# cg-tuwien/ppsurf

Hardware: AMD Instinct MI355X
Metric: occupancy query-points/sec @ res=257, 50NN (higher is better)
Workload: dtype f16x3

## Files before the change

### ppsurf_amd/csrc/pps_decode.hip

```cpp
#include <cstdlib>
#include "pps_common.h"
#include "../../include/ppsurf_amd.h"

using namespace pps;

#ifndef NT
#define NT 256
#endif
#define NW (NT / 64)
#ifndef WG_PER_CU
#define WG_PER_CU (512 / NT)
#endif
#ifndef PPS_PRIO
#define PPS_PRIO 1
#endif
#ifndef PPS_PRIO_PN
#define PPS_PRIO_PN 1
#endif
#define CH4 2048

template <int CHUNK_F4_NEXT, int NTH = NT, class F>
__device__ __forceinline__ void stream_step(const f32x4* __restrict__ gnext, f32x4*& cur, f32x4*& nxt, F&& compute) {
    chunk_copy_async<CHUNK_F4_NEXT / NTH, NTH>(gnext, nxt);
    compute((const f32x4*)cur);
// ... 799 lines not shown
                           [&](const f32x4* w) { dense_blocks<8, 4, 1>(h, u[t], w, bias_g + 32, lane); });
        }
#pragma unroll 1
        for (int c = 0; c < 32; ++c) {
            f32x4 o[PB_T][8];
            const f32x4* gn = (c + 1 < 32) ? wg + (6 + c) * CH4 : wg;
            stream_step<CH4>(gn, cur, nxt, [&](const f32x4* w) {
#pragma unroll
                for (int t = 0; t < PB_T; ++t) dense_blocks<4, 8, 0>(u[t], o[t], w, bias4 + 32 * c, lane);
            });
#pragma unroll
            for (int t = 0; t < PB_T; ++t) {
                if (qvs[t]) {
                    f32x4* dst = (f32x4*)(trans2 + qcs[t] * 4096) + g;
#pragma unroll
                    for (int j = 0; j < 8; ++j) dst[4 * (8 * c + j)] = o[t][j];
                }
            }
        }
    }
}

__global__ __launch_bounds__(NT, 2) void pointnet_stn_fc_h_kernel(const float* __restrict__ gin, int64_t Q, const f32x4* __restrict__ w16,
                                                                  const float* __restrict__ bias, half8* __restrict__ trans2h, int* __restrict__ range) {
    float amax = 0.f;
    f32x4* buf0 = (f32x4*)pps_smem;
    f32x4* buf1 = buf0 + CH4;
    float* bias_l = (float*)(buf1 + CH4);
    const f32x4* bias4 = (const f32x4*)bias_l;
    const f32x4* wg = w16;
    const int lane = lane_id(), wave = threadIdx.x >> 6, n = lane & 15, g = lane >> 4;

    lds_fill(bias_l, bias + 192, 4096);
    const f32x4* bias_g = (const f32x4*)bias;
    stream_prologue<CH4>(wg, buf0);
    stream_wait();
    __syncthreads();
    f32x4 *cur = buf0, *nxt = buf1;
    const int ntiles = (int)((Q + NW * 16 - 1) / (NW * 16));
    int first, count, stride;
    xcd_tile_range(ntiles, first, count, stride);
    for (int it = 0; it < count; ++it) {
        const int64_t qi = (int64_t)(first + it * stride) * (NW * 16) + wave * 16 + n;
        const bool qv = qi < Q;
        const int64_t qc = qv ? qi : Q - 1;
        HiLo ah[8], h[4], u[2];
        {
            f32x4 a[16];
            const f32x4* src = (const f32x4*)(gin + qc * 256) + g;
#pragma unroll
            for (int bb = 0; bb < 16; ++bb) a[bb] = src[4 * bb];
#pragma unroll
            for (int kb = 0; kb < 8; ++kb) ah[kb] = split_f16_r(amax, a[2 * kb], a[2 * kb + 1]);
        }
#pragma unroll
        for (int c = 0; c < 4; ++c)
            stream_step<CH4>(wg + (c + 1) * CH4, cur, nxt, [&](const f32x4* w) {
                dense_blocks_f16x3<8, 2, 1>(ah, (const half8*)w, bias_g + 8 * c, lane, [&](int, const f32x4& o0, const f32x4& o1) { h[c] = split_f16_r(amax, o0, o1); }); });
        stream_step<CH4>(wg + 5 * CH4, cur, nxt, [&](const f32x4* w) {
            dense_blocks_f16x3<4, 4, 1>(h, (const half8*)w, bias_g + 32, lane, [&](int i, const f32x4& o0, const f32x4& o1) { u[i] = split_f16_r(amax, o0, o1); }); });
        half8* dst = trans2h + qc * 1024 + g;
#pragma unroll 1
        for (int c = 0; c < 32; ++c) {
            const f32x4* gn = (c + 1 < 32) ? wg + (6 + c) * CH4 : wg;
            stream_step<CH4>(gn, cur, nxt, [&](const f32x4* w) {
                dense_blocks_f16x3<2, 8, 0, false>(u, (const half8*)w, bias4 + 32 * c, lane, [&](int i, const f32x4& o0, const f32x4& o1) {
                    const int a = 2 * c + (i >> 1), kb = i & 1;
                    const HiLo v = split_f16_r(amax, o0, o1);
                    if (qv) {
                        half8* d = dst + (((a >> 4) * 2 + kb) * 2) * 64 + 4 * (a & 15);
                        d[0] = v.hi;
                        d[64] = v.lo;
                    }
                }); });
        }
    }
    range_commit(amax, range);
}

#define PC_W_XYZ 256
#define PC_NBIAS (576 + 256 + 4)
#define PC_WFLOATS (4096 + 8192)
#define PC_LDS_BYTES ((PC_WFLOATS + PC_W_XYZ + PC_NBIAS) * 4)

template <bool H>
__global__ __launch_bounds__(PNT, 2) void pointnet_feat_rows_kernel(const float* __restrict__ patches, const float* __restrict__ trans2,
                                                                    int64_t Q, int P, const float* __restrict__ wpack,
                                                                    const f32x4* __restrict__ wdense, const float* __restrict__ bias,
                                                                    float* __restrict__ xbar, int* __restrict__ flag) {
    if (!H && gate_closed(flag)) return;
    float amax = 0.f;
    f32x4* w_l = (f32x4*)pps_smem;
    float* xyz_l = (float*)(w_l + PC_WFLOATS / 4);
    float* bias_l = xyz_l + PC_W_XYZ;
    const f32x4* bias4 = (const f32x4*)bias_l;
    const f32x4* u4 = bias4 + 144;
    const int lane = lane_id(), wave = threadIdx.x >> 6, n = lane & 15, g = lane >> 4;
    for (int i = threadIdx.x; i < PC_WFLOATS / 4; i += PNT) w_l[i] = wdense[i];
    lds_fill(xyz_l, wpack, PC_W_XYZ);
    lds_fill(bias_l, bias, PC_NBIAS);
    __syncthreads();
    const float s0 = bias_l[576 + 256];
    const f32x4* w_c0b = w_l;
    const f32x4* w_c2 = w_l + 1024;
    const int ntile_rows = (P + 15) / 16;

    const int ntiles = (int)((Q + PNW - 1) / PNW);
    int first, count, stride;
    xcd_tile_range(ntiles, first, count, stride);
    for (int it = 0; it < count; ++it) {
        const int64_t q = (int64_t)(first + it * stride) * PNW + wave;
        if (q >= Q) continue;
        half8 th[4][2], tl[4][2];
        f32x4 tf[4][4];
        if (H) {
            const half8* tq = (const half8*)trans2 + q * 1024 + 4 * n + g;
#pragma unroll
            for (int ob = 0; ob < 4; ++ob)
#pragma unroll
                for (int kb = 0; kb < 2; ++kb) { th[ob][kb] = tq[((ob * 2 + kb) * 2) * 64]; tl[ob][kb] = tq[((ob * 2 + kb) * 2 + 1) * 64]; }
        } else {
            const f32x4* tq = (const f32x4*)(trans2 + q * 4096);
#pragma unroll
            for (int ob = 0; ob < 4; ++ob)
#pragma unroll
                for (int kb = 0; kb < 4; ++kb) tf[ob][kb] = tq[(16 * ob + n) * 16 + 4 * kb + g];
        }
        f32x4 acc[8];
        float mrun = -INFINITY, ssum = 0.f;
#pragma unroll
        for (int bb = 0; bb < 8; ++bb) acc[bb] = f32x4{0.f, 0.f, 0.f, 0.f};
        for (int rb = 0; rb < ntile_rows; ++rb) {
            const int rowi = rb * 16 + n;
            const bool valid = rowi < P;
            const int rowc = valid ? rowi : P - 1;
            const float coord = (g < 3) ? patches[(q * P + rowc) * 3 + g] : 0.f;
            f32x4 x0[4], y[8];
#pragma unroll
            for (int bb = 0; bb < 4; ++bb) x0[bb] = bias4[4 * bb + g];
            xyz_blocks<4>(coord, x0, xyz_l, lane);
            relu_blocks<4>(x0);
            __builtin_amdgcn_s_setprio(PPS_PRIO_PN);
            float s = 0.f;
            if (H) {
                HiLo a[2], b[2];
                a[0] = split_f16_r(amax, x0[0], x0[1]);
                a[1] = split_f16_r(amax, x0[2], x0[3]);
                dense_blocks_f16x3<2, 4, 1>(a, (const half8*)w_c0b, bias4 + 16, lane, [&](int i, const f32x4& o0, const f32x4& o1) { b[i] = split_f16_r(amax, o0, o1); });
#pragma unroll
                for (int ob = 0; ob < 4; ++ob) {
                    f32x4 o = bias4[32 + 4 * ob + g], c = {0.f, 0.f, 0.f, 0.f};
#pragma unroll
                    for (int kb = 0; kb < 2; ++kb) {
                        o = __builtin_amdgcn_mfma_f32_16x16x32_f16(th[ob][kb], b[kb].hi, o, 0, 0, 0);
                        c = __builtin_amdgcn_mfma_f32_16x16x32_f16(th[ob][kb], b[kb].lo, c, 0, 0, 0);
                        c = __builtin_amdgcn_mfma_f32_16x16x32_f16(tl[ob][kb], b[kb].hi, c, 0, 0, 0);
                    }
                    o += c;
#pragma unroll
                    for (int r = 0; r < 4; ++r) x0[ob][r] = fmaxf(o[r], 0.f);
                }
                a[0] = split_f16_r(amax, x0[0], x0[1]);
                a[1] = split_f16_r(amax, x0[2], x0[3]);
                dense_blocks_f16x3<2, 8, 1>(a, (const half8*)w_c2, bias4 + 48, lane, [&](int i, const f32x4& o0, const f32x4& o1) {
                    const f32x4 w0 = u4[4 * (2 * i) + g], w1 = u4[4 * (2 * i + 1) + g];
#pragma unroll
                    for (int r = 0; r < 4; ++r) s += w0[r] * o0[r] + w1[r] * o1[r];
                    y[2 * i] = o0;
                    y[2 * i + 1] = o1;
                });
            } else {
                f32x4 x1[4];
                dense_blocks<4, 4, 1>(x0, x1, w_c0b, bias4 + 16, lane);
#pragma unroll
                for (int ob = 0; ob < 4; ++ob) {
                    f32x4 o = bias4[32 + 4 * ob + g];
#pragma unroll
                    for (int kb = 0; kb < 4; ++kb) {
                        o = __builtin_amdgcn_mfma_f32_16x16x4f32(tf[ob][kb].x, x1[kb].x, o, 0, 0, 0);
                        o = __builtin_amdgcn_mfma_f32_16x16x4f32(tf[ob][kb].y, x1[kb].y, o, 0, 0, 0);
                        o = __builtin_amdgcn_mfma_f32_16x16x4f32(tf[ob][kb].z, x1[kb].z, o, 0, 0, 0);
                        o = __builtin_amdgcn_mfma_f32_16x16x4f32(tf[ob][kb].w, x1[kb].w, o, 0, 0, 0);
                    }
#pragma unroll
                    for (int r = 0; r < 4; ++r) x0[ob][r] = fmaxf(o[r], 0.f);
                }
                dense_blocks<4, 8, 1>(x0, y, w_c2, bias4 + 48, lane);
#pragma unroll
                for (int bb = 0; bb < 8; ++bb) {
                    const f32x4 w4 = u4[4 * bb + g];
#pragma unroll
                    for (int r = 0; r < 4; ++r) s += w4[r] * y[bb][r];
                }
            }
            __builtin_amdgcn_s_setprio(0);
            s += __shfl_xor(s, 16);
            s += __shfl_xor(s, 32);
            s += s0;
            const float mblk = row16_max(valid ? s : -INFINITY);
            const float mnew = fmaxf(mrun, mblk);
            const float scale = __expf(mrun - mnew);
            const float en = valid ? __expf(s - mnew) : 0.f;
            mrun = mnew;
            ssum = ssum * scale + en;
#pragma unroll
            for (int bb = 0; bb < 8; ++bb)
#pragma unroll
                for (int r = 0; r < 4; ++r) acc[bb][r] = acc[bb][r] * scale + en * y[bb][r];
        }
        const float inv = 1.f / row16_sum(ssum);
        rows16_sum_transposed8(acc, lane);
        if (n < 8) ((f32x4*)(xbar + q * 128))[4 * n + g] = acc[0] * inv;
    }
    if (H) range_commit(amax, flag);
}

#define TL_NBIAS (256 + 256 + 32)
#define TL_LDS_BYTES (2 * CH4 * 16 + TL_NBIAS * 4)

__global__ __launch_bounds__(NT, 2) void decode_tail_kernel(const float* __restrict__ pooled, const float* __restrict__ xbar, int64_t Q,
                                                            const float* __restrict__ wpack, const float* __restrict__ bias,
                                                            float* __restrict__ logits, float* __restrict__ occ, int* __restrict__ gate) {
    if (gate_closed(gate)) return;
    if (gate != nullptr && blockIdx.x == 0 && threadIdx.x == 0) atomicAdd(gate + 1, 1);
    f32x4* buf0 = (f32x4*)pps_smem;
    f32x4* buf1 = buf0 + CH4;
    float* bias_l = (float*)(buf1 + CH4);
    const f32x4* bias4 = (const f32x4*)bias_l;
    const f32x4* wg = (const f32x4*)wpack;
    const int lane = lane_id(), wave = threadIdx.x >> 6, n = lane & 15, g = lane >> 4;

    lds_fill(bias_l, bias, TL_NBIAS);
    stream_prologue<CH4>(wg, buf0);
    stream_wait();
    __syncthreads();
    f32x4 *cur = buf0, *nxt = buf1;

    const int ntiles = (int)((Q + NW * 16 - 1) / (NW * 16));
    int first, count, stride;
    xcd_tile_range(ntiles, first, count, stride);
    for (int it = 0; it < count; ++it) {
        const int64_t qi = (int64_t)(first + it * stride) * (NW * 16) + wave * 16 + n;
        const bool qv = qi < Q;
        const int64_t qc = qv ? qi : Q - 1;
        f32x4 p[16], x[8], h[16];
        {
            const f32x4* sp = (const f32x4*)(pooled + qc * 256) + g;
            const f32x4* sx = (const f32x4*)(xbar + qc * 128) + g;
#pragma unroll
            for (int bb = 0; bb < 16; ++bb) p[bb] = sp[4 * bb];
#pragma unroll
            for (int bb = 0; bb < 8; ++bb) x[bb] = sx[4 * bb];
        }
#pragma unroll
        for (int c = 0; c < 8; ++c)
            stream_step<CH4>(wg + (c + 1) * CH4, cur, nxt,
                           [&](const f32x4* w) { dense_blocks<16, 2, 0>(p, &h[2 * c], w, bias4 + 8 * c, lane); });
#pragma unroll
        for (int c = 0; c < 4; ++c)
            stream_step<CH4>(wg + (c + 9) * CH4, cur, nxt,
                           [&](const f32x4* w) { dense_blocks<8, 4, 1, 1>(x, &h[4 * c], w, bias4, lane); });
#pragma unroll
        for (int c = 0; c < 8; ++c)
            stream_step<CH4>(wg + (c + 13) * CH4, cur, nxt,
                           [&](const f32x4* w) { dense_blocks<16, 2, 1>(h, &p[2 * c], w, bias4 + 64 + 8 * c, lane); });
        f32x4 o[2];
        stream_step<CH4>(wg, cur, nxt, [&](const f32x4* w) { dense_blocks<16, 2, 0>(p, o, w, bias4 + 128, lane); });
        if (qv && g == 0) {
            const float l0 = o[0].x, l1 = o[0].y;
            logits[qi * 2] = l0;
            logits[qi * 2 + 1] = l1;
            if (occ) {
                const float mx = fmaxf(l0, l1);
                const float e0 = __expf(l0 - mx), e1 = __expf(l1 - mx);
                occ[qi] = (e0 - e1) / (e0 + e1);
            }
        }
    }
}

__global__ __launch_bounds__(NT, 2) void decode_tail_h_kernel(const float* __restrict__ pooled, const float* __restrict__ xbar, int64_t Q,
                                                              const f32x4* __restrict__ w16, const float* __restrict__ bias,
                                                              float* __restrict__ logits, float* __restrict__ occ, int* __restrict__ range) {
    float amax = 0.f;
    f32x4* buf0 = (f32x4*)pps_smem;
    f32x4* buf1 = buf0 + CH4;
    float* bias_l = (float*)(buf1 + CH4);
    const f32x4* bias4 = (const f32x4*)bias_l;
    const f32x4* wg = w16;
    const int lane = lane_id(), wave = threadIdx.x >> 6, n = lane & 15, g = lane >> 4;

    lds_fill(bias_l, bias, TL_NBIAS);
    stream_prologue<CH4>(wg, buf0);
    stream_wait();
    __syncthreads();
    f32x4 *cur = buf0, *nxt = buf1;

// ... 20 lines not shown
            stream_step<CH4 / 2>(wg + c * 3072 + 2048, cur, nxt, [&](const f32x4* w) {
                dense_blocks_f16x3<8, 2, 0>(p, (const half8*)w, bias4 + 8 * c, lane, [&](int, const f32x4& o0, const f32x4& o1) { h[0] = o0; h[1] = o1; }); });
            stream_step<CH4>(c + 1 < 8 ? wg + (c + 1) * 3072 : wg + 24576, cur, nxt, [&](const f32x4* w) {
                dense_blocks_f16x3<4, 2, 1, true, true>(x, (const half8*)w, bias4, lane, [&](int, const f32x4& o0, const f32x4& o1) { y[c] = split_f16_r(amax, o0, o1); }, h); });
        }
#pragma unroll
        for (int c = 0; c < 8; ++c)
            stream_step<CH4>(wg + 24576 + (c + 1) * 2048, cur, nxt, [&](const f32x4* w) {
                dense_blocks_f16x3<8, 2, 1>(y, (const half8*)w, bias4 + 64 + 8 * c, lane, [&](int, const f32x4& o0, const f32x4& o1) { p[c] = split_f16_r(amax, o0, o1); }); });
        f32x4 o[2];
        stream_step<CH4>(wg, cur, nxt, [&](const f32x4* w) {
            dense_blocks_f16x3<8, 2, 0>(p, (const half8*)w, bias4 + 128, lane, [&](int, const f32x4& o0, const f32x4& o1) { o[0] = o0; o[1] = o1; }); });
        if (qv && g == 0) {
            const float l0 = o[0].x, l1 = o[0].y;
            logits[qi * 2] = l0;
            logits[qi * 2 + 1] = l1;
            if (occ) {
                const float mx = fmaxf(l0, l1);
                const float e0 = __expf(l0 - mx), e1 = __expf(l1 - mx);
                occ[qi] = (e0 - e1) / (e0 + e1);
            }
        }
    }
    range_commit(amax, range);
}

static int g_cu_count = 0;
static int cu_count() {
    if (g_cu_count == 0) {
        int dev = 0;
        hipDeviceProp_t prop;
        if (hipGetDevice(&dev) != hipSuccess || hipGetDeviceProperties(&prop, dev) != hipSuccess) return -1;
        g_cu_count = prop.multiProcessorCount;
    }
    return g_cu_count;
}

template <class K>
static int set_lds(K kernel, int bytes) {
    return hipFuncSetAttribute((const void*)kernel, hipFuncAttributeMaxDynamicSharedMemorySize, bytes) == hipSuccess ? 0 : 1;
}

static int grid_for(int64_t ntiles) {
    int cus = cu_count();
    if (cus <= 0) cus = 256;
    cus *= WG_PER_CU;
    return (int)(ntiles < cus ? (ntiles > 0 ? ntiles : 1) : cus);
}

struct PnSplit { int64_t q_packed; int grid_packed, grid_rest, rest_mode; };
static PnSplit pn_split(int64_t q, int p) {
    int cus = cu_count();
    if (cus <= 0) cus = 256;
    const PatchPacking pk = patch_packing(p);
    PnSplit sp;
    const int wgs = cus * PN_WG_PER_CU;
    const int64_t per_round = (int64_t)wgs * PNW * pk.qg;
    sp.q_packed = pk.packed ? (q / per_round) * per_round : 0;
    if (pk.packed && getenv("PPS_PN_FORCE_PACK")) sp.q_packed = q;
    sp.grid_packed = wgs;
    sp.rest_mode = pk.packed ? 2 : 0;
    const int64_t rest_tiles = (q - sp.q_packed + PNW - 1) / PNW;
    sp.grid_rest = (int)(rest_tiles < wgs ? rest_tiles : wgs);
    return sp;
}

#define PPS_LAUNCH_CHECK() (hipGetLastError() == hipSuccess ? PPS_OK : PPS_ERR_LAUNCH)

template <bool H>
static int launch_stn_rows(const float* patches, int64_t q, int p, const float* wpack, const void* wdense, const float* bias, float* g,
                           int* flag, void* stream) {
    static int once = set_lds(pointnet_stn_rows_kernel<H>, PA_LDS_BYTES);
    (void)once;
    const PnSplit sp = pn_split(q, p);
    if (sp.q_packed > 0)
        hipLaunchKernelGGL(pointnet_stn_rows_kernel<H>, dim3(sp.grid_packed), dim3(PNT), PA_LDS_BYTES, (hipStream_t)stream, patches,
                           sp.q_packed, p, 1, wpack, (const f32x4*)wdense, bias, g, flag);
    if (q > sp.q_packed)
        hipLaunchKernelGGL(pointnet_stn_rows_kernel<H>, dim3(sp.grid_rest), dim3(PNT), PA_LDS_BYTES, (hipStream_t)stream,
                           patches + sp.q_packed * p * 3, q - sp.q_packed, p, sp.rest_mode, wpack, (const f32x4*)wdense, bias, g + sp.q_packed * 256, flag);
    return PPS_LAUNCH_CHECK();
}

template <bool H>
static int launch_feat_rows(const float* patches, const float* trans2, int64_t q, int p, const float* wpack, const void* wdense,
                            const float* bias, float* xbar, int* flag, void* stream) {
    static int once = set_lds(pointnet_feat_rows_kernel<H>, PC_LDS_BYTES);
    (void)once;
    int cus = cu_count();
    if (cus <= 0) cus = 256;
    const int64_t ntiles = (q + PNW - 1) / PNW, wgs = (int64_t)cus * PN_WG_PER_CU;
    hipLaunchKernelGGL(pointnet_feat_rows_kernel<H>, dim3((unsigned)(ntiles < wgs ? ntiles : wgs)), dim3(PNT), PC_LDS_BYTES, (hipStream_t)stream, patches,
                       trans2, q, p, wpack, (const f32x4*)wdense, bias, xbar, flag);
    return PPS_LAUNCH_CHECK();
}


static int interp_pool_f32_impl(const float* G, const float* pts, const float* query, const int64_t* idx, int64_t q, int k,
                                const float* wpack, const float* bias, float* pooled, const int* gate, void* stream) {
    if (q < 0 || k < 1 || k > 64) return PPS_ERR_ARG;
    if (q == 0) return PPS_OK;
    if (!G || !pts || !query || !idx || !wpack || !bias || !pooled) return PPS_ERR_ARG;
    static int once = set_lds(interp_pool_kernel, IP_LDS_BYTES);
    (void)once;
    hipLaunchKernelGGL(interp_pool_kernel, dim3(grid_for((q + NW / 4 - 1) / (NW / 4))), dim3(NT), IP_LDS_BYTES, (hipStream_t)stream,
                       G, pts, query, idx, q, k, wpack, bias, pooled, gate);
    return PPS_LAUNCH_CHECK();
}

static int stn_fc_f32_impl(const float* g, int64_t q, const float* wpack, const float* bias, float* trans2, const int* gate, void* stream) {
    if (q < 0) return PPS_ERR_ARG;
    if (q == 0) return PPS_OK;
    if (!g || !wpack || !bias || !trans2) return PPS_ERR_ARG;
    static int once = set_lds(pointnet_stn_fc_kernel, PB_LDS_BYTES);
    (void)once;
    hipLaunchKernelGGL(pointnet_stn_fc_kernel, dim3(grid_for((q + NW * 16 * PB_T - 1) / (NW * 16 * PB_T))), dim3(NT), PB_LDS_BYTES, (hipStream_t)stream,
                       g, q, wpack, bias, trans2, gate);
    return PPS_LAUNCH_CHECK();
}

static int decode_tail_f32_impl(const float* pooled, const float* xbar, int64_t q, const float* wpack, const float* bias,
                                float* logits, float* occ, int* gate, void* stream) {
    if (q < 0) return PPS_ERR_ARG;
    if (q == 0) return PPS_OK;
    if (!pooled || !xbar || !wpack || !bias || !logits) return PPS_ERR_ARG;
    static int once = set_lds(decode_tail_kernel, TL_LDS_BYTES);
    (void)once;
    hipLaunchKernelGGL(decode_tail_kernel, dim3(grid_for((q + NW * 16 - 1) / (NW * 16))), dim3(NT), TL_LDS_BYTES, (hipStream_t)stream,
                       pooled, xbar, q, wpack, bias, logits, occ, gate);
    return PPS_LAUNCH_CHECK();
}

extern "C" {

int pps_abi_version(void) { return 2; }

int pps_debug_occupancy(int which) {
    int n = -1;
    if (which == 0) { set_lds(interp_pool_kernel, IP_LDS_BYTES); hipOccupancyMaxActiveBlocksPerMultiprocessor(&n, interp_pool_kernel, NT, IP_LDS_BYTES); }
    if (which == 1) { set_lds(pointnet_stn_rows_kernel<false>, PA_LDS_BYTES); hipOccupancyMaxActiveBlocksPerMultiprocessor(&n, pointnet_stn_rows_kernel<false>, PNT, PA_LDS_BYTES); }
    if (which == 3) { set_lds(pointnet_stn_fc_kernel, PB_LDS_BYTES); hipOccupancyMaxActiveBlocksPerMultiprocessor(&n, pointnet_stn_fc_kernel, NT, PB_LDS_BYTES); }
    if (which == 4) { set_lds(pointnet_stn_fc_h_kernel, PB_LDS_BYTES); hipOccupancyMaxActiveBlocksPerMultiprocessor(&n, pointnet_stn_fc_h_kernel, NT, PB_LDS_BYTES); }
    if (which == 2) { set_lds(pointnet_feat_rows_kernel<false>, PC_LDS_BYTES); hipOccupancyMaxActiveBlocksPerMultiprocessor(&n, pointnet_feat_rows_kernel<false>, PNT, PC_LDS_BYTES); }
    return n;
}
int pps_device_cu_count(void) { return cu_count(); }

int pps_rows_dense256_f32(const float* in, int64_t rs, int64_t cs, int64_t m, const float* wpack, const float* bias,
                          float* out, void* stream) {
    if (m < 0) return PPS_ERR_ARG;
    if (m == 0) return PPS_OK;
    if (!in || !wpack || !bias || !out) return PPS_ERR_ARG;
    if (cs == 1 && (rs % 4) != 0) return PPS_ERR_ARG;
    static int once = set_lds(rows_dense256_kernel, RD_LDS_BYTES);
    (void)once;
    hipLaunchKernelGGL(rows_dense256_kernel, dim3(grid_for((m + NW * 16 - 1) / (NW * 16))), dim3(NT), RD_LDS_BYTES, (hipStream_t)stream,
                       in, rs, cs, m, wpack, bias, out);
    return PPS_LAUNCH_CHECK();
}

int pps_interp_pool_f32(const float* G, const float* pts, const float* query, const int64_t* idx, int64_t q, int k,
                        const float* wpack, const float* bias, float* pooled, void* stream) {
    return interp_pool_f32_impl(G, pts, query, idx, q, k, wpack, bias, pooled, nullptr, stream);
}

int pps_interp_pool_f16x3(const float* G, const float* pts, const float* query, const int64_t* idx, int64_t q, int k,
                          const float* wxyz, const void* w16, const float* bias, float* pooled, int32_t* range_flag, void* stream) {
    if (q < 0 || k < 1 || k > 64) return PPS_ERR_ARG;
    if (q == 0) return PPS_OK;
    if (!G || !pts || !query || !idx || !wxyz || !w16 || !bias || !pooled) return PPS_ERR_ARG;
    static int once = set_lds(interp_pool_f16x3_kernel, IH_LDS_BYTES);
    (void)once;
    int cus = cu_count();
    if (cus <= 0) cus = 256;
    const int64_t ntiles = (q + IH_NW / 4 - 1) / (IH_NW / 4);
    const int64_t wgs = (int64_t)cus * IH_WG_PER_CU;
    const int grid = (int)(ntiles < wgs ? ntiles : wgs);
    hipLaunchKernelGGL(interp_pool_f16x3_kernel, dim3(grid), dim3(IH_NT), IH_LDS_BYTES, (hipStream_t)stream,
                       G, pts, query, idx, q, k, wxyz, (const f32x4*)w16, bias, pooled, (int*)range_flag);
    return PPS_LAUNCH_CHECK();
}

int pps_interp_small_f32(const float* G, const float* pts, const float* query, const int64_t* idx, int64_t q, int k, int c,
                         const float* wpack, const float* bias, const float* wtail, int nout, float* out, void* stream) {
    if (q < 0 || k < 1 || k > 64 || (c != 32 && c != 64) || nout < 1 || nout > IS_MAX_OUT) return PPS_ERR_ARG;
    if (q == 0) return PPS_OK;
    if (!G || !pts || !query || !idx || !wpack || !bias || !wtail || !out) return PPS_ERR_ARG;
    int cus = cu_count();
    if (cus <= 0) cus = 256;
    const int grid = (int)(q < (int64_t)cus * 8 ? q : (int64_t)cus * 8);
    hipStream_t st = (hipStream_t)stream;
    if (c == 32) hipLaunchKernelGGL((interp_small_kernel<2, false>), dim3(grid), dim3(IS_NT), 0, st, G, pts, query, idx, q, k, wpack, nullptr, bias, wtail, nout, out, nullptr);
    else hipLaunchKernelGGL((interp_small_kernel<4, false>), dim3(grid), dim3(IS_NT), 0, st, G, pts, query, idx, q, k, wpack, nullptr, bias, wtail, nout, out, nullptr);
    return PPS_LAUNCH_CHECK();
}

int pps_interp_small_f16x3(const float* G, const float* pts, const float* query, const int64_t* idx, int64_t q, int k, int c,
                           const float* wpack, const void* w16, const float* bias, const float* wtail, int nout, float* out, int* guard,
                           void* stream) {
    if (q < 0 || k < 1 || k > 64 || (c != 32 && c != 64) || nout < 1 || nout > IS_MAX_OUT) return PPS_ERR_ARG;
    if (q == 0) return PPS_OK;
    if (!G || !pts || !query || !idx || !wpack || !w16 || !bias || !wtail || !out || !guard) return PPS_ERR_ARG;
    int cus = cu_count();
    if (cus <= 0) cus = 256;
    const int grid = (int)(q < (int64_t)cus * 8 ? q : (int64_t)cus * 8);
    hipStream_t st = (hipStream_t)stream;
    if (hipMemsetAsync(guard, 0, sizeof(int), st) != hipSuccess) return PPS_ERR_LAUNCH;
    const float* wh = (const float*)w16;
    if (c == 32) {
        hipLaunchKernelGGL((interp_small_kernel<2, true>), dim3(grid), dim3(IS_NT), 0, st, G, pts, query, idx, q, k, wpack, wh, bias, wtail, nout, out, guard);
        hipLaunchKernelGGL((interp_small_kernel<2, false>), dim3(grid), dim3(IS_NT), 0, st, G, pts, query, idx, q, k, wpack, nullptr, bias, wtail, nout, out, guard);
    } else {
        hipLaunchKernelGGL((interp_small_kernel<4, true>), dim3(grid), dim3(IS_NT), 0, st, G, pts, query, idx, q, k, wpack, wh, bias, wtail, nout, out, guard);
        hipLaunchKernelGGL((interp_small_kernel<4, false>), dim3(grid), dim3(IS_NT), 0, st, G, pts, query, idx, q, k, wpack, nullptr, bias, wtail, nout, out, guard);
    }
    return PPS_LAUNCH_CHECK();
}

int pps_pointnet_stn_rows_f32(const float* patches, int64_t q, int p, const float* wpack, const float* bias, float* g,
                              void* stream) {
    if (q < 0 || p < 1) return PPS_ERR_ARG;
    if (q == 0) return PPS_OK;
    if (!patches || !wpack || !bias || !g) return PPS_ERR_ARG;
    return launch_stn_rows<false>(patches, q, p, wpack, wpack + PA_W_XYZ, bias, g, nullptr, stream);
}

int pps_pointnet_stn_fc_f32(const float* g, int64_t q, const float* wpack, const float* bias, float* trans2, void* stream) {
    return stn_fc_f32_impl(g, q, wpack, bias, trans2, nullptr, stream);
}

int pps_pointnet_feat_rows_f32(const float* patches, const float* trans2, int64_t q, int p, const float* wpack,
                               const float* bias, float* xbar, void* stream) {
    if (q < 0 || p < 1) return PPS_ERR_ARG;
    if (q == 0) return PPS_OK;
    if (!patches || !trans2 || !wpack || !bias || !xbar) return PPS_ERR_ARG;
    return launch_feat_rows<false>(patches, trans2, q, p, wpack, wpack + PC_W_XYZ, bias, xbar, nullptr, stream);
}

int pps_pointnet_f16x3(const float* patches, int64_t q, int p, const float* const* weights ,
                       const void* const* w16, float* g, float* trans2, float* xbar, int32_t* range_flag, void* const* events, void* stream) {
    if (q < 0 || p < 1) return PPS_ERR_ARG;
    if (q == 0) return PPS_OK;
    if (!patches || !weights || !w16 || !w16[0] || !w16[1] || !w16[2] || !g || !trans2 || !xbar) return PPS_ERR_ARG;
    hipStream_t st = (hipStream_t)stream;
    int* range = (int*)range_flag;
    int rc = launch_stn_rows<true>(patches, q, p, weights[0], w16[0], weights[1], g, range, stream);
    if (events && events[0]) hipEventRecord((hipEvent_t)events[0], st);
    if (rc != PPS_OK) return rc;
    static int once = set_lds(pointnet_stn_fc_h_kernel, PB_LDS_BYTES);
    (void)once;
    static const int64_t sub = getenv("PPS_PN_SUB") ? atoll(getenv("PPS_PN_SUB")) : 0;
    static const bool reuse = getenv("PPS_PN_SUB_REUSE") != nullptr;
    if (sub > 0 && sub < q) {
        for (int64_t off = 0; off < q && rc == PPS_OK; off += sub) {
            const int64_t n = q - off < sub ? q - off : sub;
            float* t2 = reuse ? trans2 : trans2 + off * 4096;
            hipLaunchKernelGGL(pointnet_stn_fc_h_kernel, dim3(grid_for((n + NW * 16 - 1) / (NW * 16))), dim3(NT), PB_LDS_BYTES, st, g + off * 256, n,
                               (const f32x4*)w16[1], weights[3], (half8*)t2, range);
            rc = launch_feat_rows<true>(patches + off * p * 3, t2, n, p, weights[4], w16[2], weights[5], xbar + off * 128, range, stream);
        }
        if (events && events[1]) hipEventRecord((hipEvent_t)events[1], st);
        if (events && events[2]) hipEventRecord((hipEvent_t)events[2], st);
        return rc;
    }
    hipLaunchKernelGGL(pointnet_stn_fc_h_kernel, dim3(grid_for((q + NW * 16 - 1) / (NW * 16))), dim3(NT), PB_LDS_BYTES, st, g, q,
                       (const f32x4*)w16[1], weights[3], (half8*)trans2, range);
    if (events && events[1]) hipEventRecord((hipEvent_t)events[1], st);
    if (hipGetLastError() != hipSuccess) return PPS_ERR_LAUNCH;
    rc = launch_feat_rows<true>(patches, trans2, q, p, weights[4], w16[2], weights[5], xbar, range, stream);
    if (events && events[2]) hipEventRecord((hipEvent_t)events[2], st);
    return rc;
}

int pps_decode_tail_f32(const float* pooled, const float* xbar, int64_t q, const float* wpack, const float* bias,
                        float* logits, float* occ, void* stream) {
    return decode_tail_f32_impl(pooled, xbar, q, wpack, bias, logits, occ, nullptr, stream);
}

int pps_decode_tail_f16x3(const float* pooled, const float* xbar, int64_t q, const void* w16, const float* bias, float* logits, float* occ,
                          int32_t* range_flag, void* stream) {
    if (q < 0) return PPS_ERR_ARG;
    if (q == 0) return PPS_OK;
    if (!pooled || !xbar || !w16 || !bias || !logits) return PPS_ERR_ARG;
    static int once = set_lds(decode_tail_h_kernel, TL_LDS_BYTES);
    (void)once;
    hipLaunchKernelGGL(decode_tail_h_kernel, dim3(grid_for((q + NW * 16 - 1) / (NW * 16))), dim3(NT), TL_LDS_BYTES, (hipStream_t)stream,
                       pooled, xbar, q, (const f32x4*)w16, bias, logits, occ, (int*)range_flag);
    return PPS_LAUNCH_CHECK();
}

#define PPS_DECODE_WS_HEAD 64
size_t pps_decode_ws_bytes(int64_t q) { return q < 0 ? 0 : (size_t)q * (256 + 256 + 4096 + 256) * sizeof(float) + PPS_DECODE_WS_HEAD; }

static int decode_fwd(const float* table, const float* pts, const float* query, const int64_t* idx, int64_t q, int k,
                      const float* patches, int p, const float* const* weights, float* logits, float* occ, void* ws, void* const* events,
                      void* stream, const void* const* w16 = nullptr) {
    const void* interp_w16 = w16 ? w16[0] : nullptr;
    const bool pn16 = w16 && w16[1] && w16[2] && w16[3];
    if (q < 0) return PPS_ERR_ARG;
    if (q == 0) return PPS_OK;
    if (!weights || !ws || !logits) return PPS_ERR_ARG;
    for (int i = 0; i < 10; ++i)
        if (!weights[i]) return PPS_ERR_ARG;
    int* guard = (int*)ws;
    float* pooled = (float*)ws + PPS_DECODE_WS_HEAD / sizeof(float);
    float* g = pooled + q * 256;
    float* trans2 = g + q * 256;
    float* xbar = trans2 + q * 4096;
    hipStream_t st = (hipStream_t)stream;
    const bool split = interp_w16 || pn16 || (w16 && w16[4]);
    if (split && hipMemsetAsync(guard, 0, sizeof(int), st) != hipSuccess) return PPS_ERR_LAUNCH;
#define PPS_MARK(i) do { if (events && events[i] && hipEventRecord((hipEvent_t)events[i], st) != hipSuccess) return PPS_ERR_LAUNCH; } while (0)
    PPS_MARK(0);
    int rc = interp_w16 ? pps_interp_pool_f16x3(table, pts, query, idx, q, k, weights[0], interp_w16, weights[1], pooled, guard, stream)
                        : pps_interp_pool_f32(table, pts, query, idx, q, k, weights[0], weights[1], pooled, stream);
    PPS_MARK(1);
    if (pn16) {
        if (rc == PPS_OK) rc = pps_pointnet_f16x3(patches, q, p, weights + 2, w16 + 1, g, trans2, xbar, guard, events ? events + 2 : nullptr, stream);
    } else {
        if (rc == PPS_OK) rc = pps_pointnet_stn_rows_f32(patches, q, p, weights[2], weights[3], g, stream);
        PPS_MARK(2);
        if (rc == PPS_OK) rc = pps_pointnet_stn_fc_f32(g, q, weights[4], weights[5], trans2, stream);
        PPS_MARK(3);
        if (rc == PPS_OK) rc = pps_pointnet_feat_rows_f32(patches, trans2, q, p, weights[6], weights[7], xbar, stream);
        PPS_MARK(4);
    }
    if (rc == PPS_OK)
        rc = (w16 && w16[4]) ? pps_decode_tail_f16x3(pooled, xbar, q, w16[4], weights[9], logits, occ, guard, stream)
                             : pps_decode_tail_f32(pooled, xbar, q, weights[8], weights[9], logits, occ, stream);
    PPS_MARK(5);
#undef PPS_MARK
    if (split && rc == PPS_OK) {
        rc = interp_pool_f32_impl(table, pts, query, idx, q, k, weights[0], weights[1], pooled, guard, stream);
        if (rc == PPS_OK) rc = launch_stn_rows<false>(patches, q, p, weights[2], weights[2] + PA_W_XYZ, weights[3], g, guard, stream);
        if (rc == PPS_OK) rc = stn_fc_f32_impl(g, q, weights[4], weights[5], trans2, guard, stream);
        if (rc == PPS_OK) rc = launch_feat_rows<false>(patches, trans2, q, p, weights[6], weights[6] + PC_W_XYZ, weights[7], xbar, guard, stream);
        if (rc == PPS_OK) rc = decode_tail_f32_impl(pooled, xbar, q, weights[8], weights[9], logits, occ, guard, stream);
    }
    return rc;
}

int pps_decode_fwd_f32(const float* table, const float* pts, const float* query, const int64_t* idx, int64_t q, int k,
                       const float* patches, int p, const float* const* weights, float* logits, float* occ, void* ws, void* stream) {
    return decode_fwd(table, pts, query, idx, q, k, patches, p, weights, logits, occ, ws, nullptr, stream);
}

int pps_decode_fwd_events_f32(const float* table, const float* pts, const float* query, const int64_t* idx, int64_t q, int k,
                              const float* patches, int p, const float* const* weights, float* logits, float* occ, void* ws,
                              void* const* events, void* stream) {
    return decode_fwd(table, pts, query, idx, q, k, patches, p, weights, logits, occ, ws, events, stream);
}

int pps_decode_fwd_mixed_f32(const float* table, const float* pts, const float* query, const int64_t* idx, int64_t q, int k,
                             const float* patches, int p, const float* const* weights, const void* const* w16, float* logits, float* occ,
// ... 7 lines not shown
```

Baseline: 12.58 million.

## Prefetch next patch coords and transform matrix across rows in feat kernel

Adds a prefetch variant of the split-precision pointnet feature kernel. It issues the next row block's coordinate load, and on the last row block the next query's transform-matrix load, early via inline asm global loads with hand-placed s_waitcnt. The aim is to hide global load latency behind the MFMA work. The variant is on by default and can be disabled with an environment variable. It relies on exact vmcnt counting (vmcnt(17)), which is fragile and adds register pressure from holding the prefetched matrix.

```diff
diff --git a/ppsurf_amd/csrc/pps_decode.hip b/ppsurf_amd/csrc/pps_decode.hip
--- a/ppsurf_amd/csrc/pps_decode.hip
+++ b/ppsurf_amd/csrc/pps_decode.hip
@@ -906,7 +906,7 @@
 #define PC_WFLOATS (4096 + 8192)
 #define PC_LDS_BYTES ((PC_WFLOATS + PC_W_XYZ + PC_NBIAS) * 4)
 
-template <bool H>
+template <bool H, bool PF = false>
 __global__ __launch_bounds__(PNT, 2) void pointnet_feat_rows_kernel(const float* __restrict__ patches, const float* __restrict__ trans2,
                                                                     int64_t Q, int P, const float* __restrict__ wpack,
                                                                     const f32x4* __restrict__ wdense, const float* __restrict__ bias,
@@ -931,17 +931,43 @@
     const int ntiles = (int)((Q + PNW - 1) / PNW);
     int first, count, stride;
     xcd_tile_range(ntiles, first, count, stride);
+    static_assert(H || !PF, "the early placement exists for the split-precision kernel only");
+    half8 th[4][2], tl[4][2];
+    float cnext = 0.f;
+    bool held = false;
+#define PC_LOAD_M(qq)                                                                                                                       \
+    {                                                                                                                                       \
+        int64_t slot = (qq) * 1024 + 4 * n + g;                                                                                             \
+        if (PF) asm volatile("" : "+v"(slot));         \
+        const half8* tq = PF ? (const half8*)trans2 + slot : (const half8*)trans2 + (qq) * 1024 + 4 * n + g;                                \
+        _Pragma("unroll") for (int ob = 0; ob < 4; ++ob)                                                                                    \
+            _Pragma("unroll") for (int kb = 0; kb < 2; ++kb) {                                                                              \
+                th[ob][kb] = tq[((ob * 2 + kb) * 2) * 64];                                                                                  \
+                tl[ob][kb] = tq[((ob * 2 + kb) * 2 + 1) * 64];                                                                              \
+            }                                                                                                                               \
+    }
+    auto coord_request = [&](int64_t qq, int rb) {
+        const int ri = rb * 16 + n;
+        const float* src = patches + (qq * P + (ri < P ? ri : P - 1)) * 3 + (g < 3 ? g : 2);
+        float v;
+        asm volatile("global_load_dword %0, %1, off" : "=v"(v) : "v"(src) : "memory");
+        return v;
+    };
     for (int it = 0; it < count; ++it) {
         const int64_t q = (int64_t)(first + it * stride) * PNW + wave;
-        if (q >= Q) continue;
-        half8 th[4][2], tl[4][2];
+        if (q >= Q) { held = false; continue; }
+        const int64_t qn = (int64_t)(first + (it + 1) * stride) * PNW + wave;
+        const bool has_next = PF && it + 1 < count && qn < Q;
         f32x4 tf[4][4];
-        if (H) {
-            const half8* tq = (const half8*)trans2 + q * 1024 + 4 * n + g;
-#pragma unroll
-            for (int ob = 0; ob < 4; ++ob)
-#pragma unroll
-                for (int kb = 0; kb < 2; ++kb) { th[ob][kb] = tq[((ob * 2 + kb) * 2) * 64]; tl[ob][kb] = tq[((ob * 2 + kb) * 2 + 1) * 64]; }
+        const bool steady = held;
+        if (H && PF) {
+            if (!held) {
+                cnext = coord_request(q, 0);
+                PC_LOAD_M(q)
+                asm volatile("s_waitcnt vmcnt(0)" : "+v"(cnext), "+v"(tl[3][1]));
+            }
+        } else if (H) {
+            PC_LOAD_M(q)
         } else {
             const f32x4* tq = (const f32x4*)(trans2 + q * 4096);
 #pragma unroll
@@ -957,7 +983,14 @@
             const int rowi = rb * 16 + n;
             const bool valid = rowi < P;
             const int rowc = valid ? rowi : P - 1;
-            const float coord = (g < 3) ? patches[(q * P + rowc) * 3 + g] : 0.f;
+            float coord;
+            if (PF) {
+                if (rb == 0 && steady) asm volatile("s_waitcnt vmcnt(17)" : "+v"(cnext));
+                else asm volatile("s_waitcnt vmcnt(0)" : "+v"(cnext));
+                coord = (g < 3) ? cnext : 0.f;
+            } else {
+                coord = (g < 3) ? patches[(q * P + rowc) * 3 + g] : 0.f;
+            }
             f32x4 x0[4], y[8];
 #pragma unroll
             for (int bb = 0; bb < 4; ++bb) x0[bb] = bias4[4 * bb + g];
@@ -982,6 +1015,12 @@
                     o += c;
 #pragma unroll
                     for (int r = 0; r < 4; ++r) x0[ob][r] = fmaxf(o[r], 0.f);
+                }
+                if (PF) {
+                    const bool last = rb + 1 == ntile_rows;
+                    __builtin_amdgcn_sched_barrier(0);
+                    cnext = coord_request(last && has_next ? qn : q, last ? (has_next ? 0 : rb) : rb + 1);
+                    if (last && has_next) PC_LOAD_M(qn)
                 }
                 a[0] = split_f16_r(amax, x0[0], x0[1]);
                 a[1] = split_f16_r(amax, x0[2], x0[3]);
@@ -1034,7 +1073,9 @@
         const float inv = 1.f / row16_sum(ssum);
         rows16_sum_transposed8(acc, lane);
         if (n < 8) ((f32x4*)(xbar + q * 128))[4 * n + g] = acc[0] * inv;
-    }
+        held = has_next;
+    }
+#undef PC_LOAD_M
     if (H) range_commit(amax, flag);
 }
 
@@ -1222,17 +1263,32 @@
     return PPS_LAUNCH_CHECK();
 }
 
-template <bool H>
-static int launch_feat_rows(const float* patches, const float* trans2, int64_t q, int p, const float* wpack, const void* wdense,
-                            const float* bias, float* xbar, int* flag, void* stream) {
-    static int once = set_lds(pointnet_feat_rows_kernel<H>, PC_LDS_BYTES);
+static bool& feat_rows_prefetch() {
+    static bool on = [] {
+        const char* e = getenv("PPS_FEAT_PREFETCH");
+        return !(e && atoi(e) == 0);
+    }();
+    return on;
+}
+
+template <bool H, bool PF>
+static int launch_feat_rows_pf(const float* patches, const float* trans2, int64_t q, int p, const float* wpack, const void* wdense,
+                               const float* bias, float* xbar, int* flag, void* stream) {
+    static int once = set_lds(pointnet_feat_rows_kernel<H, PF>, PC_LDS_BYTES);
     (void)once;
     int cus = cu_count();
     if (cus <= 0) cus = 256;
     const int64_t ntiles = (q + PNW - 1) / PNW, wgs = (int64_t)cus * PN_WG_PER_CU;
-    hipLaunchKernelGGL(pointnet_feat_rows_kernel<H>, dim3((unsigned)(ntiles < wgs ? ntiles : wgs)), dim3(PNT), PC_LDS_BYTES, (hipStream_t)stream, patches,
-                       trans2, q, p, wpack, (const f32x4*)wdense, bias, xbar, flag);
+    hipLaunchKernelGGL((pointnet_feat_rows_kernel<H, PF>), dim3((unsigned)(ntiles < wgs ? ntiles : wgs)), dim3(PNT), PC_LDS_BYTES, (hipStream_t)stream,
+                       patches, trans2, q, p, wpack, (const f32x4*)wdense, bias, xbar, flag);
     return PPS_LAUNCH_CHECK();
+}
+
+template <bool H>
+static int launch_feat_rows(const float* patches, const float* trans2, int64_t q, int p, const float* wpack, const void* wdense,
+                            const float* bias, float* xbar, int* flag, void* stream) {
+    if (H && feat_rows_prefetch()) return launch_feat_rows_pf<H, H>(patches, trans2, q, p, wpack, wdense, bias, xbar, flag, stream);
+    return launch_feat_rows_pf<H, false>(patches, trans2, q, p, wpack, wdense, bias, xbar, flag, stream);
 }
 
 
@@ -1281,8 +1337,14 @@
     if (which == 1) { set_lds(pointnet_stn_rows_kernel<false>, PA_LDS_BYTES); hipOccupancyMaxActiveBlocksPerMultiprocessor(&n, pointnet_stn_rows_kernel<false>, PNT, PA_LDS_BYTES); }
     if (which == 3) { set_lds(pointnet_stn_fc_kernel, PB_LDS_BYTES); hipOccupancyMaxActiveBlocksPerMultiprocessor(&n, pointnet_stn_fc_kernel, NT, PB_LDS_BYTES); }
     if (which == 4) { set_lds(pointnet_stn_fc_h_kernel, PB_LDS_BYTES); hipOccupancyMaxActiveBlocksPerMultiprocessor(&n, pointnet_stn_fc_h_kernel, NT, PB_LDS_BYTES); }
-    if (which == 2) { set_lds(pointnet_feat_rows_kernel<false>, PC_LDS_BYTES); hipOccupancyMaxActiveBlocksPerMultiprocessor(&n, pointnet_feat_rows_kernel<false>, PNT, PC_LDS_BYTES); }
+    if (which == 2) { set_lds(pointnet_feat_rows_kernel<false, false>, PC_LDS_BYTES); hipOccupancyMaxActiveBlocksPerMultiprocessor(&n, pointnet_feat_rows_kernel<false, false>, PNT, PC_LDS_BYTES); }
     return n;
+}
+int ppsdbg_feat_rows_prefetch(int on) {
+    bool& flag = feat_rows_prefetch();
+    const int was = flag ? 1 : 0;
+    if (on >= 0) flag = on > 0;
+    return was;
 }
 int pps_device_cu_count(void) { return cu_count(); }
 
```

After: 12.65 million (median of 6 runs). About the same (+0.5%).

## Fuse STN fc3 transform generation into PointNet feature-rows kernel via LDS

Applied to the files above, without the earlier changes.

Splits the STN MLP into a head kernel that writes only a small 32-wide intermediate, then fuses the final fc3 layer (which produces the per-query 64x64 transform) into the feature-rows kernel. The transform is written to LDS and consumed there instead of going through a large global trans2 buffer. This removes heavy global write and read traffic. In exchange it uses 512-thread blocks with a much larger LDS footprint, extra barriers, and fc3 weights re-read per 16-query tile. The old path stays available through PPS_PN_FUSED=0.

```diff
diff --git a/ppsurf_amd/csrc/pps_decode.hip b/ppsurf_amd/csrc/pps_decode.hip
--- a/ppsurf_amd/csrc/pps_decode.hip
+++ b/ppsurf_amd/csrc/pps_decode.hip
@@ -905,6 +905,99 @@
 #define PC_NBIAS (576 + 256 + 4)
 #define PC_WFLOATS (4096 + 8192)
 #define PC_LDS_BYTES ((PC_WFLOATS + PC_W_XYZ + PC_NBIAS) * 4)
+
+template <bool H>
+__device__ __forceinline__ void feat_rows_query(const float* __restrict__ patches, int64_t q, int P, int ntile_rows, const half8 (&th)[4][2],
+                                                const half8 (&tl)[4][2], const f32x4 (&tf)[4][4], const f32x4* bias4, const f32x4* u4,
+                                                const float* xyz_l, const f32x4* w_c0b, const f32x4* w_c2, float s0, float& amax, int lane,
+                                                float* __restrict__ xbar) {
+    const int n = lane & 15, g = lane >> 4;
+    f32x4 acc[8];
+    float mrun = -INFINITY, ssum = 0.f;
+#pragma unroll
+    for (int bb = 0; bb < 8; ++bb) acc[bb] = f32x4{0.f, 0.f, 0.f, 0.f};
+    for (int rb = 0; rb < ntile_rows; ++rb) {
+        const int rowi = rb * 16 + n;
+        const bool valid = rowi < P;
+        const int rowc = valid ? rowi : P - 1;
+        const float coord = (g < 3) ? patches[(q * P + rowc) * 3 + g] : 0.f;
+        f32x4 x0[4], y[8];
+#pragma unroll
+        for (int bb = 0; bb < 4; ++bb) x0[bb] = bias4[4 * bb + g];
+        xyz_blocks<4>(coord, x0, xyz_l, lane);
+        relu_blocks<4>(x0);
+        __builtin_amdgcn_s_setprio(PPS_PRIO_PN);
+        float s = 0.f;
+        if (H) {
+            HiLo a[2], b[2];
+            a[0] = split_f16_r(amax, x0[0], x0[1]);
+            a[1] = split_f16_r(amax, x0[2], x0[3]);
+            dense_blocks_f16x3<2, 4, 1>(a, (const half8*)w_c0b, bias4 + 16, lane, [&](int i, const f32x4& o0, const f32x4& o1) { b[i] = split_f16_r(amax, o0, o1); });
+#pragma unroll
+            for (int ob = 0; ob < 4; ++ob) {
+                f32x4 o = bias4[32 + 4 * ob + g], c = {0.f, 0.f, 0.f, 0.f};
+#pragma unroll
+                for (int kb = 0; kb < 2; ++kb) {
+                    o = __builtin_amdgcn_mfma_f32_16x16x32_f16(th[ob][kb], b[kb].hi, o, 0, 0, 0);
+                    c = __builtin_amdgcn_mfma_f32_16x16x32_f16(th[ob][kb], b[kb].lo, c, 0, 0, 0);
+                    c = __builtin_amdgcn_mfma_f32_16x16x32_f16(tl[ob][kb], b[kb].hi, c, 0, 0, 0);
+                }
+                o += c;
+#pragma unroll
+                for (int r = 0; r < 4; ++r) x0[ob][r] = fmaxf(o[r], 0.f);
+            }
+            a[0] = split_f16_r(amax, x0[0], x0[1]);
+            a[1] = split_f16_r(amax, x0[2], x0[3]);
+            dense_blocks_f16x3<2, 8, 1>(a, (const half8*)w_c2, bias4 + 48, lane, [&](int i, const f32x4& o0, const f32x4& o1) {
+                const f32x4 w0 = u4[4 * (2 * i) + g], w1 = u4[4 * (2 * i + 1) + g];
+#pragma unroll
+                for (int r = 0; r < 4; ++r) s += w0[r] * o0[r] + w1[r] * o1[r];
+                y[2 * i] = o0;
+                y[2 * i + 1] = o1;
+            });
+        } else {
+            f32x4 x1[4];
+            dense_blocks<4, 4, 1>(x0, x1, w_c0b, bias4 + 16, lane);
+#pragma unroll
+            for (int ob = 0; ob < 4; ++ob) {
+                f32x4 o = bias4[32 + 4 * ob + g];
+#pragma unroll
+                for (int kb = 0; kb < 4; ++kb) {
+                    o = __builtin_amdgcn_mfma_f32_16x16x4f32(tf[ob][kb].x, x1[kb].x, o, 0, 0, 0);
+                    o = __builtin_amdgcn_mfma_f32_16x16x4f32(tf[ob][kb].y, x1[kb].y, o, 0, 0, 0);
+                    o = __builtin_amdgcn_mfma_f32_16x16x4f32(tf[ob][kb].z, x1[kb].z, o, 0, 0, 0);
+                    o = __builtin_amdgcn_mfma_f32_16x16x4f32(tf[ob][kb].w, x1[kb].w, o, 0, 0, 0);
+                }
+#pragma unroll
+                for (int r = 0; r < 4; ++r) x0[ob][r] = fmaxf(o[r], 0.f);
+            }
+            dense_blocks<4, 8, 1>(x0, y, w_c2, bias4 + 48, lane);
+#pragma unroll
+            for (int bb = 0; bb < 8; ++bb) {
+                const f32x4 w4 = u4[4 * bb + g];
+#pragma unroll
+                for (int r = 0; r < 4; ++r) s += w4[r] * y[bb][r];
+            }
+        }
+        __builtin_amdgcn_s_setprio(0);
+        s += __shfl_xor(s, 16);
+        s += __shfl_xor(s, 32);
+        s += s0;
+        const float mblk = row16_max(valid ? s : -INFINITY);
+        const float mnew = fmaxf(mrun, mblk);
+        const float scale = __expf(mrun - mnew);
+        const float en = valid ? __expf(s - mnew) : 0.f;
+        mrun = mnew;
+        ssum = ssum * scale + en;
+#pragma unroll
+        for (int bb = 0; bb < 8; ++bb)
+#pragma unroll
+            for (int r = 0; r < 4; ++r) acc[bb][r] = acc[bb][r] * scale + en * y[bb][r];
+    }
+    const float inv = 1.f / row16_sum(ssum);
+    rows16_sum_transposed8(acc, lane);
+    if (n < 8) ((f32x4*)(xbar + q * 128))[4 * n + g] = acc[0] * inv;
+}
 
 template <bool H>
 __global__ __launch_bounds__(PNT, 2) void pointnet_feat_rows_kernel(const float* __restrict__ patches, const float* __restrict__ trans2,
@@ -949,93 +1042,137 @@
 #pragma unroll
                 for (int kb = 0; kb < 4; ++kb) tf[ob][kb] = tq[(16 * ob + n) * 16 + 4 * kb + g];
         }
-        f32x4 acc[8];
-        float mrun = -INFINITY, ssum = 0.f;
-#pragma unroll
-        for (int bb = 0; bb < 8; ++bb) acc[bb] = f32x4{0.f, 0.f, 0.f, 0.f};
-        for (int rb = 0; rb < ntile_rows; ++rb) {
-            const int rowi = rb * 16 + n;
-            const bool valid = rowi < P;
-            const int rowc = valid ? rowi : P - 1;
-            const float coord = (g < 3) ? patches[(q * P + rowc) * 3 + g] : 0.f;
-            f32x4 x0[4], y[8];
-#pragma unroll
-            for (int bb = 0; bb < 4; ++bb) x0[bb] = bias4[4 * bb + g];
-            xyz_blocks<4>(coord, x0, xyz_l, lane);
-            relu_blocks<4>(x0);
-            __builtin_amdgcn_s_setprio(PPS_PRIO_PN);
-            float s = 0.f;
-            if (H) {
-                HiLo a[2], b[2];
-                a[0] = split_f16_r(amax, x0[0], x0[1]);
-                a[1] = split_f16_r(amax, x0[2], x0[3]);
-                dense_blocks_f16x3<2, 4, 1>(a, (const half8*)w_c0b, bias4 + 16, lane, [&](int i, const f32x4& o0, const f32x4& o1) { b[i] = split_f16_r(amax, o0, o1); });
-#pragma unroll
-                for (int ob = 0; ob < 4; ++ob) {
-                    f32x4 o = bias4[32 + 4 * ob + g], c = {0.f, 0.f, 0.f, 0.f};
-#pragma unroll
-                    for (int kb = 0; kb < 2; ++kb) {
-                        o = __builtin_amdgcn_mfma_f32_16x16x32_f16(th[ob][kb], b[kb].hi, o, 0, 0, 0);
-                        c = __builtin_amdgcn_mfma_f32_16x16x32_f16(th[ob][kb], b[kb].lo, c, 0, 0, 0);
-                        c = __builtin_amdgcn_mfma_f32_16x16x32_f16(tl[ob][kb], b[kb].hi, c, 0, 0, 0);
+        feat_rows_query<H>(patches, q, P, ntile_rows, th, tl, tf, bias4, u4, xyz_l, w_c0b, w_c2, s0, amax, lane, xbar);
+    }
+    if (H) range_commit(amax, flag);
+}
+
+#define PH_LDS_BYTES (2 * CH4 * 16)
+__global__ __launch_bounds__(NT, 2) void pointnet_stn_head_h_kernel(const float* __restrict__ gin, int64_t Q, const f32x4* __restrict__ w16,
+                                                                    const float* __restrict__ bias, half8* __restrict__ uh, int* __restrict__ range) {
+    float amax = 0.f;
+    f32x4* buf0 = (f32x4*)pps_smem;
+    f32x4* buf1 = buf0 + CH4;
+    const f32x4* wg = w16;
+    const int lane = lane_id(), wave = threadIdx.x >> 6, n = lane & 15, g = lane >> 4;
+    const f32x4* bias_g = (const f32x4*)bias;
+    stream_prologue<CH4>(wg, buf0);
+    stream_wait();
+    __syncthreads();
+    f32x4 *cur = buf0, *nxt = buf1;
+    const int ntiles = (int)((Q + NW * 16 - 1) / (NW * 16));
+    int first, count, stride;
+    xcd_tile_range(ntiles, first, count, stride);
+    for (int it = 0; it < count; ++it) {
+        const int64_t qi = (int64_t)(first + it * stride) * (NW * 16) + wave * 16 + n;
+        const bool qv = qi < Q;
+        const int64_t qc = qv ? qi : Q - 1;
+        HiLo ah[8], h[4], u[2];
+        {
+            f32x4 a[16];
+            const f32x4* src = (const f32x4*)(gin + qc * 256) + g;
+#pragma unroll
+            for (int bb = 0; bb < 16; ++bb) a[bb] = src[4 * bb];
+#pragma unroll
+            for (int kb = 0; kb < 8; ++kb) ah[kb] = split_f16_r(amax, a[2 * kb], a[2 * kb + 1]);
+        }
+#pragma unroll
+        for (int c = 0; c < 4; ++c)
+            stream_step<CH4>(wg + (c + 1) * CH4, cur, nxt, [&](const f32x4* w) {
+                dense_blocks_f16x3<8, 2, 1>(ah, (const half8*)w, bias_g + 8 * c, lane, [&](int, const f32x4& o0, const f32x4& o1) { h[c] = split_f16_r(amax, o0, o1); }); });
+        stream_step<CH4>(wg, cur, nxt, [&](const f32x4* w) {
+            dense_blocks_f16x3<4, 4, 1>(h, (const half8*)w, bias_g + 32, lane, [&](int i, const f32x4& o0, const f32x4& o1) { u[i] = split_f16_r(amax, o0, o1); }); });
+        if (qv) {
+            half8* dst = uh + qc * 16 + g;
+#pragma unroll
+            for (int kb = 0; kb < 2; ++kb) { dst[(2 * kb) * 4] = u[kb].hi; dst[(2 * kb + 1) * 4] = u[kb].lo; }
+        }
+    }
+    range_commit(amax, range);
+}
+
+#define PF_NT 512
+#define PF_QSTRIDE 257
+#define PF_BUF (8 * PF_QSTRIDE)
+#define PF_LDS_BYTES (PC_LDS_BYTES + 3 * PF_BUF * 16)
+__global__ __launch_bounds__(PF_NT, 2) void pointnet_fc3_feat_rows_kernel(const float* __restrict__ patches, const half8* __restrict__ uh,
+                                                                          int64_t Q, int P, const f32x4* __restrict__ wfc,
+                                                                          const float* __restrict__ bias_fc, const float* __restrict__ wpack,
+                                                                          const f32x4* __restrict__ wdense, const float* __restrict__ bias,
+                                                                          float* __restrict__ xbar, int* __restrict__ flag) {
+    float amax = 0.f;
+    f32x4* w_l = (f32x4*)pps_smem;
+    float* xyz_l = (float*)(w_l + PC_WFLOATS / 4);
+    float* bias_l = xyz_l + PC_W_XYZ;
+    half8* ex = (half8*)(bias_l + PC_NBIAS);
+    const f32x4* bias4 = (const f32x4*)bias_l;
+    const f32x4* u4 = bias4 + 144;
+    const int lane = lane_id(), wave = __builtin_amdgcn_readfirstlane(threadIdx.x >> 6), n = lane & 15, g = lane >> 4;
+    for (int i = threadIdx.x; i < PC_WFLOATS / 4; i += PF_NT) w_l[i] = wdense[i];
+    lds_fill(xyz_l, wpack, PC_W_XYZ);
+    lds_fill(bias_l, bias, PC_NBIAS);
+    const float s0 = bias[576 + 256];
+    const f32x4* w_c0b = w_l;
+    const f32x4* w_c2 = w_l + 1024;
+    const int ntile_rows = (P + 15) / 16;
+    const f32x4* w3 = wfc + 5 * CH4;
+    const f32x4* b3 = (const f32x4*)(bias_fc + 192);
+    half8* ex_w = ex + (n < 8 ? n * PF_QSTRIDE : PF_BUF + (n - 8) * PF_QSTRIDE) + 8 * wave + g;
+    const half8* ex_r = ex + wave * PF_QSTRIDE + 4 * n + g;
+    const half8* ex_r2 = ex_r + PF_BUF;
+
+    const int ntiles = (int)((Q + 15) / 16);
+    int first, count, stride;
+    xcd_tile_range(ntiles, first, count, stride);
+    const f32x4 tf[4][4] = {};
+    for (int it = 0; it < count; ++it) {
+        const int64_t q0 = (int64_t)(first + it * stride) * 16;
+        half8 th[4][2], tl[4][2], th2[2][2], tl2[2][2];
+        {
+            const int64_t qc = q0 + n < Q ? q0 + n : Q - 1;
+            HiLo u[2];
+#pragma unroll
+            for (int kb = 0; kb < 2; ++kb) { u[kb].hi = uh[qc * 16 + (2 * kb) * 4 + g]; u[kb].lo = uh[qc * 16 + (2 * kb + 1) * 4 + g]; }
+#pragma unroll
+            for (int ob = 0; ob < 4; ++ob) {
+                __syncthreads();
+                const int c = 8 * ob + wave;
+                const half8* wc = (const half8*)(w3 + c * CH4);
+                asm volatile("" : "+s"(wc));
+                dense_blocks_f16x3<2, 8, 0, false>(u, wc, b3 + 32 * c, lane, [&](int i, const f32x4& o0, const f32x4& o1) {
+                    const HiLo v = split_f16_r(amax, o0, o1);
+                    half8* d = ex_w + (n >= 8 ? (ob & 1) * PF_BUF : 0) + ((i & 1) * 2) * 64 + 4 * (i >> 1);
+                    d[0] = v.hi;
+                    d[64] = v.lo;
+                });
+                __syncthreads();
+#pragma unroll
+                for (int kb = 0; kb < 2; ++kb) {
+                    th[ob][kb] = ex_r[(2 * kb) * 64];
+                    tl[ob][kb] = ex_r[(2 * kb + 1) * 64];
+                    if (ob < 2) {
+                        th2[ob][kb] = ex_r2[ob * PF_BUF + (2 * kb) * 64];
+                        tl2[ob][kb] = ex_r2[ob * PF_BUF + (2 * kb + 1) * 64];
                     }
-                    o += c;
-#pragma unroll
-                    for (int r = 0; r < 4; ++r) x0[ob][r] = fmaxf(o[r], 0.f);
                 }
-                a[0] = split_f16_r(amax, x0[0], x0[1]);
-                a[1] = split_f16_r(amax, x0[2], x0[3]);
-                dense_blocks_f16x3<2, 8, 1>(a, (const half8*)w_c2, bias4 + 48, lane, [&](int i, const f32x4& o0, const f32x4& o1) {
-                    const f32x4 w0 = u4[4 * (2 * i) + g], w1 = u4[4 * (2 * i + 1) + g];
-#pragma unroll
-                    for (int r = 0; r < 4; ++r) s += w0[r] * o0[r] + w1[r] * o1[r];
-                    y[2 * i] = o0;
-                    y[2 * i + 1] = o1;
-                });
-            } else {
-                f32x4 x1[4];
-                dense_blocks<4, 4, 1>(x0, x1, w_c0b, bias4 + 16, lane);
-#pragma unroll
-                for (int ob = 0; ob < 4; ++ob) {
-                    f32x4 o = bias4[32 + 4 * ob + g];
-#pragma unroll
-                    for (int kb = 0; kb < 4; ++kb) {
-                        o = __builtin_amdgcn_mfma_f32_16x16x4f32(tf[ob][kb].x, x1[kb].x, o, 0, 0, 0);
-                        o = __builtin_amdgcn_mfma_f32_16x16x4f32(tf[ob][kb].y, x1[kb].y, o, 0, 0, 0);
-                        o = __builtin_amdgcn_mfma_f32_16x16x4f32(tf[ob][kb].z, x1[kb].z, o, 0, 0, 0);
-                        o = __builtin_amdgcn_mfma_f32_16x16x4f32(tf[ob][kb].w, x1[kb].w, o, 0, 0, 0);
-                    }
-#pragma unroll
-                    for (int r = 0; r < 4; ++r) x0[ob][r] = fmaxf(o[r], 0.f);
+            }
+        }
+        if (q0 + wave < Q) feat_rows_query<true>(patches, q0 + wave, P, ntile_rows, th, tl, tf, bias4, u4, xyz_l, w_c0b, w_c2, s0, amax, lane, xbar);
+        if (q0 + wave + 8 < Q) {
+#pragma unroll
+            for (int kb = 0; kb < 2; ++kb) {
+#pragma unroll
+                for (int ob = 0; ob < 2; ++ob) {
+                    th[ob][kb] = th2[ob][kb];
+                    tl[ob][kb] = tl2[ob][kb];
+                    th[2 + ob][kb] = ex_r2[ob * PF_BUF + (2 * kb) * 64];
+                    tl[2 + ob][kb] = ex_r2[ob * PF_BUF + (2 * kb + 1) * 64];
                 }
-                dense_blocks<4, 8, 1>(x0, y, w_c2, bias4 + 48, lane);
-#pragma unroll
-                for (int bb = 0; bb < 8; ++bb) {
-                    const f32x4 w4 = u4[4 * bb + g];
-#pragma unroll
-                    for (int r = 0; r < 4; ++r) s += w4[r] * y[bb][r];
-                }
-            }
-            __builtin_amdgcn_s_setprio(0);
-            s += __shfl_xor(s, 16);
-            s += __shfl_xor(s, 32);
-            s += s0;
-            const float mblk = row16_max(valid ? s : -INFINITY);
-            const float mnew = fmaxf(mrun, mblk);
-            const float scale = __expf(mrun - mnew);
-            const float en = valid ? __expf(s - mnew) : 0.f;
-            mrun = mnew;
-            ssum = ssum * scale + en;
-#pragma unroll
-            for (int bb = 0; bb < 8; ++bb)
-#pragma unroll
-                for (int r = 0; r < 4; ++r) acc[bb][r] = acc[bb][r] * scale + en * y[bb][r];
-        }
-        const float inv = 1.f / row16_sum(ssum);
-        rows16_sum_transposed8(acc, lane);
-        if (n < 8) ((f32x4*)(xbar + q * 128))[4 * n + g] = acc[0] * inv;
-    }
-    if (H) range_commit(amax, flag);
+            }
+            feat_rows_query<true>(patches, q0 + wave + 8, P, ntile_rows, th, tl, tf, bias4, u4, xyz_l, w_c0b, w_c2, s0, amax, lane, xbar);
+        }
+    }
+    range_commit(amax, flag);
 }
 
 #define TL_NBIAS (256 + 256 + 32)
@@ -1403,13 +1540,31 @@
         if (events && events[2]) hipEventRecord((hipEvent_t)events[2], st);
         return rc;
     }
-    hipLaunchKernelGGL(pointnet_stn_fc_h_kernel, dim3(grid_for((q + NW * 16 - 1) / (NW * 16))), dim3(NT), PB_LDS_BYTES, st, g, q,
+    const char* fused_env = getenv("PPS_PN_FUSED");
+    if (fused_env && fused_env[0] == '0' && fused_env[1] == 0) {
+        hipLaunchKernelGGL(pointnet_stn_fc_h_kernel, dim3(grid_for((q + NW * 16 - 1) / (NW * 16))), dim3(NT), PB_LDS_BYTES, st, g, q,
+                           (const f32x4*)w16[1], weights[3], (half8*)trans2, range);
+        if (events && events[1]) hipEventRecord((hipEvent_t)events[1], st);
+        if (hipGetLastError() != hipSuccess) return PPS_ERR_LAUNCH;
+        rc = launch_feat_rows<true>(patches, trans2, q, p, weights[4], w16[2], weights[5], xbar, range, stream);
+        if (events && events[2]) hipEventRecord((hipEvent_t)events[2], st);
+        return rc;
+    }
+    static int once_head = set_lds(pointnet_stn_head_h_kernel, PH_LDS_BYTES);
+    static int once_fused = set_lds(pointnet_fc3_feat_rows_kernel, PF_LDS_BYTES);
+    (void)once_head;
+    (void)once_fused;
+    hipLaunchKernelGGL(pointnet_stn_head_h_kernel, dim3(grid_for((q + NW * 16 - 1) / (NW * 16))), dim3(NT), PH_LDS_BYTES, st, g, q,
                        (const f32x4*)w16[1], weights[3], (half8*)trans2, range);
     if (events && events[1]) hipEventRecord((hipEvent_t)events[1], st);
     if (hipGetLastError() != hipSuccess) return PPS_ERR_LAUNCH;
-    rc = launch_feat_rows<true>(patches, trans2, q, p, weights[4], w16[2], weights[5], xbar, range, stream);
+    int cus = cu_count();
+    if (cus <= 0) cus = 256;
+    const int64_t passes = (q + 15) / 16;
+    hipLaunchKernelGGL(pointnet_fc3_feat_rows_kernel, dim3((unsigned)(passes < cus ? passes : cus)), dim3(PF_NT), PF_LDS_BYTES, st, patches,
+                       (const half8*)trans2, q, p, (const f32x4*)w16[1], weights[3], weights[4], (const f32x4*)w16[2], weights[5], xbar, range);
     if (events && events[2]) hipEventRecord((hipEvent_t)events[2], st);
-    return rc;
+    return PPS_LAUNCH_CHECK();
 }
 
 int pps_decode_tail_f32(const float* pooled, const float* xbar, int64_t q, const float* wpack, const float* bias,
```

New measurement: 12.77 million before, 13.09 million after (median of 6 runs). 2.5% higher.
